# alibaba/open-simulator

Hardware: AMD Instinct MI355X
Metric: capacity-plan scenarios/sec (10k pods x ~1k nodes) (higher is better)
Workload: dtype u8 score table + u32 (gcd-normalised int64 quantities) + f64 (BalancedAllocation); 1 GPU; BASELINE config 3: 10000 pods x 488..1511 nodes, 1024 node counts x 4 pod orders = 4096 scenarios (4096 per GPU); scenarios_per_gpu=4096, pods=10000, node_pool=1512, kernel=score_table

## Files before the change

### open-simulator_amd/csrc/simon_hip.hip

```cpp
#include "../../include/simon_hip.h"
#include "simon_device.h"
#include "simon_wide.h"
#include "simon_table.h"
#include "simon_subset.h"
#include "simon_podsets.h"

#include <algorithm>
#include <cstdarg>
#include <cstdio>
#include <cstdlib>
#include <cstring>
#include <map>
#include <numeric>
#include <set>
#include <tuple>
#include <string>
#include <vector>

namespace simon {
struct PodRowF { double req_c, req_m, nz_c, nz_m; int32_t cls, preset, gate; uint32_t flags; };
struct FastScalars { int32_t mask_words, Cn, Cp, P, S; uint64_t g_cpu, g_mem; const uint32_t* pod_present; int32_t pp_words; };
struct FastLaunch {
    const uint32_t *a_cpu, *a_mem; const int32_t *a_pods, *ncls; const uint32_t *i_rq_cpu, *i_rq_mem, *i_nz_cpu, *i_nz_mem;
    const int32_t* i_npods; const PodRowF* pods; const int32_t* orders; const ScenarioDesc* scen; const int32_t* perm;
// ... 2624 lines not shown

static int run_table_batch(simon_ctx* c, const BatchRoute& r, bool want_placement, bool want_slices) {
    const int S = c->S, P = c->P;
    HIP_TRY(c, c->d_ws.ensure(c->ws_total));
    if (const char* fill = getenv("SIMON_WS_FILL"))
        HIP_TRY(c, hipMemsetAsync(c->d_ws.p, atoi(fill), c->ws_total, c->stream));
    if (want_placement) HIP_TRY(c, c->d_place_step.ensure((size_t)S * P));
    TableCold cold = table_cold(c, want_slices);
    TableLaunch f{};
    f.team = r.team; f.lds_ws = r.lds_ws; f.lds_x = r.lds_x;
    f.coarse = c->table_coarse; f.rest = c->rest; f.spread = c->spread; f.aff = c->rest && !c->aff_idx.empty(); f.nzeq = c->nzeq; f.has_pin = c->has_pin;
    f.sc = table_scalars(c, want_slices);
    const bool shared_pro = !c->no_shared_prologue && c->pro_nb > 0 && !c->has_ranks && !own_nodes(c) && table_shared_prologue(f);
    if (shared_pro) {
        HIP_TRY(c, c->d_pro_image.ensure(c->pro_bytes));
        cold.pro_image = c->d_pro_image.p; cold.pro_seg = c->d_pro_seg.p; cold.pro_nb = c->pro_nb; cold.pro_n = c->max_n;
    }
    if (c->table_prof) { HIP_TRY(c, c->d_table_prof.ensure((size_t)S * 24)); HIP_TRY(c, hipMemsetAsync(c->d_table_prof.p, 0, (size_t)S * 192, c->stream)); cold.prof = c->d_table_prof.p; }
    HIP_TRY(c, c->d_table_cold.ensure(sizeof cold));
    HIP_TRY(c, hipMemcpyAsync(c->d_table_cold.p, &cold, sizeof cold, hipMemcpyHostToDevice, c->stream));
    HIP_TRY(c, hipStreamSynchronize(c->stream));
    f.cold = reinterpret_cast<const TableCold*>(c->d_table_cold.p);
    f.cls_list = c->has_ranks ? c->d_rk_ids.p : c->d_cls_list.p; f.pods = c->d_podsC.p; f.orders = c->d_orders.p; f.perm = c->d_perm.p;
    f.place_step = want_placement ? c->d_place_step.p : nullptr;
    f.ws_off = c->d_ws_off.p; f.ws = c->d_ws.p;
    if (c->debug_route) {
        char own[64] = "none";
        if (const int lo = table_entries_own_size(f)) {
            int fits = 0;
            for (int s = 0; s < S; ++s) fits += c->scen_ni[s] <= 1024 * lo;
            if (c->no_size_dispatch) snprintf(own, sizeof own, "off");
            else snprintf(own, sizeof own, "%d of %d scenarios at %d", fits, S, lo);
        }
        fprintf(stderr, "[route] unit %s nzeq %d team %d prologue %s entries/lane %d (own size: %s)\n", table_unit_name(f), (int)f.nzeq, f.team,
                shared_pro ? "shared-image" : "per-scenario", table_entries_per_lane(f), own);
    }
    trace_segmented(c, "score-table kernel, ranked instantiation");
    if (int rc = timed_launch(c, [&] {
            if (shared_pro) HIP_TRY(c, launch_table_image(f, c->pro_nb, c->stream));
            HIP_TRY(c, launch_table(f, S, r.lds, c->stream));
            if (want_placement) HIP_TRY(c, launch_unpermute(c->d_place_step.p, c->d_inv_orders.p, c->d_scen.p, S, P, c->d_place.p, c->stream));
            return (int)SIMON_OK;
        })) return rc;
    return c->table_prof ? report_table_prof(c) : SIMON_OK;
}

static int run_fast_batch(simon_ctx* c, const BatchRoute& r, bool want_placement) {
    FastLaunch f{};
    fill_register_args(c, want_placement, f);
    f.pods = c->d_podsF.p;
    f.sc = FastScalars{(c->N + 63) / 64, c->Cn, c->Cp, c->P, c->S, c->g_cpu, c->g_mem, pod_rows(c), c->pod_W};
    return timed_launch(c, [&] { HIP_TRY(c, launch_fast(f, r.T, r.slots, c->has_mask, c->nzeq, r.lds, c->stream)); return (int)SIMON_OK; });
}

static int run_narrow_batch(simon_ctx* c, const BatchRoute& r, bool want_placement) {
    NarrowArgs a{};
    fill_register_args(c, want_placement, a);
    a.pods = c->d_podsN.p;
    a.mask_words = (c->N + 63) / 64; a.Cn = c->Cn; a.Cp = c->Cp; a.P = c->P; a.S = c->S;
    a.g_cpu = c->g_cpu; a.g_mem = c->g_mem;
    a.pod_present = pod_rows(c); a.pp_words = c->pod_W;
    return timed_launch(c, [&] { HIP_TRY(c, launch_narrow(a, r.T, r.slots, c->has_mask, c->rcp_div, r.lds, c->stream)); return (int)SIMON_OK; });
}

int simon_run_loaded(simon_ctx* c, int32_t want_placement) {
    if (!c) return SIMON_EINVAL;
    if (!c->staged || c->S <= 0) return fail(c, SIMON_ESTATE, "run_loaded: no scenarios loaded");
    if (c->evict_short >= 0 && !c->sub_on)
// ... 337 lines not shown
```

### open-simulator_amd/csrc/simon_table.h

```cpp
#pragma once

#include <hip/hip_runtime.h>
#include <stdint.h>

#include "simon_device.h"

namespace simon {

struct SigRow {
    double req_c, req_m;
    double nz_c, nz_m;
    int32_t cls;
    uint32_t flags;
    int32_t pad[2];
};
static_assert(sizeof(SigRow) == 48, "SigRow must be 48 bytes");

struct ShapeRow {
    double cap_c, cap_m;
    double rc_c, rc_m;
    double rc100_c, rc100_m;
};
static_assert(sizeof(ShapeRow) == 48, "ShapeRow must be 48 bytes");

// ... 92 lines not shown
constexpr int kTableMaxNodes = 4095;
constexpr int kTableMaxNodesCoarse = 8191;
constexpr int kTableMaxPadded = 4096;
constexpr int kTableMaxPaddedCoarse = 8192;
constexpr int kTableMaxSigs = 1023;
constexpr int kTableFastSigs = 384;
constexpr size_t kTableLdsPerCU = 160 * 1024;
constexpr int kTableMaxGpuSigs = 32;
constexpr int kTableMaxXres = 32;
constexpr int kTableMaxTerms = 120;
constexpr int kSpreadMaxZoneDom = 16;
constexpr int kSpreadMaxHostTerms = 4096, kSpreadMaxZoneTerms = 1024, kSpreadMaxZoneKeys = 3;
#ifndef SIMON_SPREAD_TAB_MAX
#define SIMON_SPREAD_TAB_MAX 512
#endif
constexpr int kSpreadTabMax = SIMON_SPREAD_TAB_MAX;
#ifndef SIMON_SPREAD_TAB_MAX2
#define SIMON_SPREAD_TAB_MAX2 2048
#endif
constexpr int kSpreadTabMax2 = SIMON_SPREAD_TAB_MAX2;
constexpr int kTeamWaves = 4;
constexpr int kTeamWavesMax = 16;
constexpr int kTableMaxClasses = 64;
constexpr int kTableMaxClassesSpread = 128;
constexpr int kTableMaxClassesPlain = 256;

constexpr int kLdsSecondTable = 0x100, kLdsTeam = 0x200, kLdsCn2 = 0x400;
size_t table_lds_bytes(int K, int ni_max, int Cn, bool coarse, bool rest, int nzk = -1);
size_t table_ws_bytes(int K, int ni, bool nzeq, bool coarse, int Cn, int M, int NZ, int TH = 0, int TZ = 0);
hipError_t launch_table(const TableLaunch& a, int n_blocks, size_t lds_bytes, hipStream_t st);
const char* table_unit_name(const TableLaunch& a);
int table_entries_per_lane(const TableLaunch& a);
int table_entries_own_size(const TableLaunch& a);
bool table_shared_prologue(const TableLaunch& a);
hipError_t launch_table_image(const TableLaunch& a, int nb, hipStream_t st);
inline size_t table_ldsx_bytes(int ni_max, int M) {
    return ((((size_t)(ni_max >> 4) * M * 2) + 127) & ~(size_t)127) + (((size_t)M * 4 + 127) & ~(size_t)127) + (((size_t)ni_max * 2 + 127) & ~(size_t)127);
}
hipError_t launch_unpermute(const int32_t* place_step, const int32_t* inv_orders, const ScenarioDesc* scen, int S, int P,
                            int32_t* placement, hipStream_t st);

}
```

### open-simulator_amd/csrc/simon_table.hip

```cpp
#ifndef SIMON_TABLE_BODY_PASS
#include "simon_table.h"

#include <algorithm>
#include <type_traits>

#ifdef SIMON_TABLE_PROFILE
#define TPROF_DECL unsigned long long tp_prev = __builtin_readcyclecounter(), tp_acc[24] = {0}; tp_acc[22] = tp_prev - tp_pro0; tp_acc[23] = tp_pro2;
#define TPROF_PROLOGUE_BEGIN const unsigned long long tp_pro0 = __builtin_readcyclecounter(); unsigned long long tp_pro2 = 0;
#define TPROF_TABLE_PASS_BEGIN tp_pro2 = __builtin_readcyclecounter()
#define TPROF_TABLE_PASS_END do { asm volatile("s_waitcnt vmcnt(0) lgkmcnt(0)" ::: "memory"); tp_pro2 = __builtin_readcyclecounter() - tp_pro2; } while (0)
#define TPROF(i) do { const unsigned long long t_ = __builtin_readcyclecounter(); tp_acc[i] += t_ - tp_prev; tp_prev = t_; } while (0)
#define TPROF_WAIT_LDS asm volatile("s_waitcnt lgkmcnt(0)" ::: "memory")
#define TPROF_WAIT_MEM asm volatile("s_waitcnt vmcnt(0)" ::: "memory")
#define TPROF_WAIT_STATE(n) asm volatile("s_waitcnt vmcnt(%0)" :: "n"(n) : "memory")
#else
#define TPROF_DECL
#define TPROF_PROLOGUE_BEGIN
#define TPROF_TABLE_PASS_BEGIN do { } while (0)
#define TPROF_TABLE_PASS_END do { } while (0)
#define TPROF(i) do { } while (0)
#define TPROF_WAIT_LDS do { } while (0)
#define TPROF_WAIT_MEM do { } while (0)
#define TPROF_WAIT_STATE(n) do { } while (0)
#endif
// ... 256 lines not shown
    int32_t* __restrict__ place_step, unsigned char* ws, const TableScalars sc) {
#endif
    GPtr<const TableCold> const cold = gp(cold_);
    GPtr<const int32_t> __restrict__ const ncls = gp(cold->ncls);
    GPtr<const int32_t> __restrict__ const cls_off = gp(cold->cls_off); GPtr<const int32_t> __restrict__ const clsprefix = gp(cold->clsprefix);
    GPtr<const int32_t> __restrict__ const a_pods = gp(cold->a_pods); GPtr<const uint32_t> __restrict__ const i_rq_cpu = gp(cold->i_rq_cpu);
    GPtr<const uint32_t> __restrict__ const i_rq_mem = gp(cold->i_rq_mem); GPtr<const uint32_t> __restrict__ const i_nz_cpu = gp(cold->i_nz_cpu);
    GPtr<const uint32_t> __restrict__ const i_nz_mem = gp(cold->i_nz_mem); GPtr<const int32_t> __restrict__ const i_npods = gp(cold->i_npods);
    const SigRow* __restrict__ const sigs = cold->sigs; const ShapeRow* __restrict__ const shapes = cold->shapes;
    const ScenarioDesc* __restrict__ const scen = cold->scen; GPtr<const uint64_t> __restrict__ const static_mask = gp(cold->static_mask);
    GPtr<const int32_t> __restrict__ const simon_raw = gp(cold->simon_raw);
    extern __shared__ __attribute__((aligned(16))) unsigned char smem[];
    const int Cn = sc.Cn, Cp = sc.Cp, P = sc.P, K = sc.K;
    constexpr int UB = COARSE ? 6 : 4;
    constexpr int UNIT = 1 << UB;
    constexpr unsigned UMASK = UNIT - 1;
    constexpr int KB = COARSE ? 13 : 12;
    constexpr unsigned PMASK = (1u << KB) - 1u;
    static_assert(!REST || COARSE, "the REST path is built on the two-level layout");
    constexpr bool kCls4 = CN2 && !REST && !SPREAD;
#ifdef SIMON_REST_CNT_HBM
    constexpr bool CNT_LDS = !COARSE;
#else
    constexpr bool CNT_LDS = (!COARSE || REST) && !kCls4;
#endif
#ifdef SIMON_TIE_SPECULATE
    constexpr bool TIE_FIRST = false;
#else
    constexpr bool TIE_FIRST = REST || MANY;
#endif
    constexpr bool kStraight = !REST && !SPREAD && !MANY;
    static_assert(!(kStraight && TIE_FIRST), "the straight-line cycle defines the winner's class and record index behind the assume's loads: nothing ahead of them may read dstar / res");
    static_assert(!kStraight || NW == 1, "team mode is SPREAD: a straight-line instantiation has no helper waves");
    constexpr bool kSharedPro = kSharedPrologueTU && !COARSE && !REST && !SPREAD && !MANY && !kCls4 && !RANKED && !LDSWS && NW == 1;
    static_assert(!MANY || (KQ == 2 && COARSE && !CN2 && !LDSX), "MANY = groups of 128 signatures on the two-level layout (since round 6 also under the REST select: its rows and counters are indexed by signature already)");
    constexpr int NG = MANY ? 2 : 0;
    static_assert(!SPREAD || COARSE, "SPREAD is built on the two-level layout");
    constexpr bool RS = REST && SPREAD;
    static_assert(!RS || (!LDSX && !CN2), "REST && SPREAD: <= 64 classes");
    static_assert(!(SPREAD && MANY) || NBQ == 2, "SPREAD with more than 128 signatures: the two-blocks-per-lane instantiations only");
    static_assert(NW == 1 || SPREAD, "team mode exists for the SPREAD instantiations");
    static_assert(!CN2 || (SPREAD && !MANY && !REST) || (REST && !LDSX && !SPREAD) || (!REST && !SPREAD && !COARSE && !MANY && !LDSWS), "CN2 = two node classes per lane in spread_select (<= 128 signatures) or in rest_select (rows in HBM); without rows and walks: 129 .. 256 classes on the one-level layout (simon_table_cls4.hip)");
    constexpr int TABMAX = CN2 ? kSpreadTabMax2 : kSpreadTabMax;
    const TCarve cv = tcarve(K, sc.ni_max, Cn, COARSE, REST, SPREAD ? (sc.NZK | ((sc.static_tables & kStSpreadAff) ? 0x100 : 0) | (NW > 1 ? 0x200 : 0) | (CN2 ? 0x400 : 0)) : -1, kCls4);
    const int TH = SPREAD ? sc.TH : 0, TZ = SPREAD ? sc.TZ : 0, NZK = SPREAD ? sc.NZK : 0;
    signed char* s_zdom = (signed char*)(smem + cv.zdom);
    unsigned short* s_stash = (unsigned short*)(smem + cv.stash);
    int* s_tabi = (int*)(smem + cv.tabi);
    int* s_tab = (int*)(smem + cv.tab);
    int* s_tot = NW > 1 ? (int*)(smem + cv.tab2) : s_tab;
    int* s_xch = (int*)(smem + cv.xch);
    const int M = REST ? sc.M : 0, G = REST ? sc.G : 0, X = REST ? sc.X : 0, NZ = REST ? sc.NZ : 0;
    const int nbp = cv.nbp;
    unsigned short* s_sn = (unsigned short*)(smem + cv.sn);
    int* s_cnt = (int*)(smem + cv.cnt);
    const ShapeRow* s_shape = (const ShapeRow*)(smem + cv.shape);
    auto shape_of = [&](int d) -> ShapeRow {
        if constexpr (kCls4) {
            const double* r = (const double*)(smem + cv.shape) + 4 * d;
            return ShapeRow{r[0], r[1], r[2], r[3], 100.0 * r[2], 100.0 * r[3]};
        } else return s_shape[d];
    };
    int* s_seg = (int*)(smem + cv.seg);
    int* s_tmp = (int*)(smem + cv.tmp);
    int2* s_ext = (int2*)(smem + cv.ext);

// ... 303 lines not shown
    if constexpr (SPREAD) {
        for (int i = tid; i < (NZK > 0 ? NZK : 1) * Cn; i += TT) s_zdom[i] = NZK > 0 ? gp(cold->cls_zdom)[i] : (signed char)0;
        for (size_t i = tid; i < ((size_t)TH * ni + 3) / 4; i += TT) ((unsigned*)g_hrow)[i] = 0u;
        for (int i = tid; i < TZ * 16; i += TT) g_zcnt[i] = 0u;
        for (int i = tid; i < TH; i += TT) g_hmax[i] = 0;
    }
    asm volatile("s_waitcnt vmcnt(0)" ::: "memory");
    if constexpr (NW > 1 || kCls4) __threadfence();
    __syncthreads();
    if constexpr (NW > 1) __threadfence();

    int kk[KQ];
    bool kvalid[KQ];
    double my_req_c[KQ], my_req_m[KQ], my_nz_c[KQ], my_nz_m[KQ];
    bool my_zero[KQ];
    int my_tc[KQ];
    unsigned my_add_c[KQ], my_add_m[KQ], my_addz_c[KQ], my_addz_m[KQ], koff[KQ];
    unsigned my_greq[KQ];
    int my_gnum[KQ];
    unsigned my_dirty = 0;
#pragma unroll
    for (int q = 0; q < KQ; ++q) {
        kvalid[q] = lane + 64 * q < K;
        kk[q] = kvalid[q] ? lane + 64 * q : 0;
        const SigRow r = sigs[kk[q]];
        my_req_c[q] = r.req_c; my_req_m[q] = r.req_m; my_nz_c[q] = r.nz_c; my_nz_m[q] = r.nz_m;
        my_zero[q] = r.flags & 1u;
        if constexpr (kCls4) my_tc[q] = r.cls;
        my_greq[q] = (unsigned)r.pad[0]; my_gnum[q] = kvalid[q] ? r.pad[1] : 0;
        my_add_c[q] = (unsigned)r.req_c; my_add_m[q] = (unsigned)r.req_m;
        my_addz_c[q] = (unsigned)r.nz_c; my_addz_m[q] = (unsigned)r.nz_m;
        koff[q] = (unsigned)kk[q] * KS;
    }
    for (int j = 0; j * 64 + lane < K; ++j) my_dirty |= 1u << j;
    int cb[NBQ], bcls[NBQ], binfo[NBQ];
#pragma unroll
    for (int q = 0; q < NBQ; ++q) {
        const int b = q * 64 + lane;
        cb[q] = (((int)(PMASK >> UB)) - b) << UB;
        bcls[q] = class_of_pos(b < nun ? b * UNIT : 0);
        binfo[q] = (cls_off[bcls[q]] - s_seg[bcls[q]] + 8192) | (bcls[q] << 16);
    }

    auto winner_info = [&](int bw) -> int {
        const int l = bw & 63, h = bw >> 6;
        int info = __builtin_amdgcn_readlane(binfo[0], l);
        if (NBQ > 1) { const int i1 = __builtin_amdgcn_readlane(binfo[NBQ > 1 ? 1 : 0], l); info = h == 1 ? i1 : info; }
        if (NBQ > 2) {
            const int i2 = __builtin_amdgcn_readlane(binfo[NBQ > 2 ? 2 : 0], l), i3 = __builtin_amdgcn_readlane(binfo[NBQ > 3 ? 3 : 0], l);
            info = h == 2 ? i2 : h == 3 ? i3 : info;
        }
        return info;
    };

    auto img_base = [&](GPtr<const TableCold> cc) -> size_t {
        return (size_t)__builtin_amdgcn_readfirstlane(gp(cc->img_slot)[s]) * (size_t)cc->img_stride;
    };
    auto class_term = [&](bool inb, int rawc, int c, int dd) -> int {
        const int lo = wave_min_i32(inb ? rawc : 0x7fffffff);
        const int hi = wave_max_i32(inb ? rawc : (int)0x80000000);
        const int range = hi >= lo ? hi - lo : 0;
        const double rr = range ? 1.0 / (double)range : 0.0;
        int term = (inb && range) ? 2 * (int)__builtin_fma((double)(rawc - lo) * 100.0, rr, 0.5 * rr) : 0;
        GPtr<const TableCold> cc = cold;
        asm volatile("" : "+s"(cc));
        if (sc.static_tables & kStNa) {
// ... 10 lines not shown
        }
        if (sc.static_tables & kStAdd) term += inb ? gp(cc->add_raw)[c * Cn + dd] : 0;
        if (sc.static_tables & kStImg) term += inb ? (int)gp(cc->img)[img_base(cc) + c * Cn + dd] : 0;
        return term;
    };
    auto class_term2 = [&](bool in0, bool in1, int raw0, int raw1, int c, int d0, int d1, int& t0, int& t1) {
        const int lo = min(wave_min_i32(in0 ? raw0 : 0x7fffffff), wave_min_i32(in1 ? raw1 : 0x7fffffff));
        const int hi = max(wave_max_i32(in0 ? raw0 : (int)0x80000000), wave_max_i32(in1 ? raw1 : (int)0x80000000));
        const int range = hi >= lo ? hi - lo : 0;
        const double rr = range ? 1.0 / (double)range : 0.0;
        t0 = (in0 && range) ? 2 * (int)__builtin_fma((double)(raw0 - lo) * 100.0, rr, 0.5 * rr) : 0;
        t1 = (in1 && range) ? 2 * (int)__builtin_fma((double)(raw1 - lo) * 100.0, rr, 0.5 * rr) : 0;
        GPtr<const TableCold> cc = cold;
        if (sc.static_tables & kStNa) {
            const int a0 = gp(cc->na_raw)[c * Cn + d0], a1 = gp(cc->na_raw)[c * Cn + d1];
            const int mx = max(wave_max_i32(in0 ? a0 : 0), wave_max_i32(in1 ? a1 : 0));
            const double r = mx ? 1.0 / (double)mx : 0.0;
            t0 += (in0 && mx) ? (int)__builtin_fma((double)a0 * 100.0, r, 0.5 * r) : 0;
            t1 += (in1 && mx) ? (int)__builtin_fma((double)a1 * 100.0, r, 0.5 * r) : 0;
        }
        if (sc.static_tables & kStTt) {
            const int a0 = gp(cc->tt_raw)[c * Cn + d0], a1 = gp(cc->tt_raw)[c * Cn + d1];
            const int mx = max(wave_max_i32(in0 ? a0 : 0), wave_max_i32(in1 ? a1 : 0));
            const double r = mx ? 1.0 / (double)mx : 0.0;
            t0 += in0 ? (mx ? 100 - (int)__builtin_fma((double)a0 * 100.0, r, 0.5 * r) : 100) : 0;
            t1 += in1 ? (mx ? 100 - (int)__builtin_fma((double)a1 * 100.0, r, 0.5 * r) : 100) : 0;
        }
        if (sc.static_tables & kStAdd) { t0 += in0 ? gp(cc->add_raw)[c * Cn + d0] : 0; t1 += in1 ? gp(cc->add_raw)[c * Cn + d1] : 0; }
        if (sc.static_tables & kStImg) {
            const size_t ib = img_base(cc);
            t0 += in0 ? (int)gp(cc->img)[ib + c * Cn + d0] : 0; t1 += in1 ? (int)gp(cc->img)[ib + c * Cn + d1] : 0;
        }
    };
    auto renormalise = [&](int k, int c) {
        if (kCls4 && Cn > 128) {
            int dq[4], cnq[4], rawq[4], tq[4];
            bool inq[4];
            int lo = 0x7fffffff, hi = (int)0x80000000;
#pragma unroll
            for (int g = 0; g < 4; ++g) {
                const bool v = g * 64 + lane < Cn;
                dq[g] = v ? g * 64 + lane : 0;
                cnq[g] = g_cnt[k * Cn + dq[g]];
                rawq[g] = simon_raw[c * Cn + dq[g]];
                inq[g] = v && cnq[g] > 0;
            }
#pragma unroll
            for (int g = 0; g < 4; ++g) { lo = min(lo, inq[g] ? rawq[g] : 0x7fffffff); hi = max(hi, inq[g] ? rawq[g] : (int)0x80000000); }
            lo = wave_min_i32(lo); hi = wave_max_i32(hi);
            if (lane == 0) s_ext[k] = make_int2(lo, hi);
            const int range = hi >= lo ? hi - lo : 0;
            const double rr = range ? 1.0 / (double)range : 0.0;
#pragma unroll
            for (int g = 0; g < 4; ++g) tq[g] = (inq[g] && range) ? 2 * (int)__builtin_fma((double)(rawq[g] - lo) * 100.0, rr, 0.5 * rr) : 0;
            GPtr<const TableCold> cc = cold;
            asm volatile("" : "+s"(cc));
            if (sc.static_tables & kStNa) {
                int a[4], mx = 0;
#pragma unroll
                for (int g = 0; g < 4; ++g) a[g] = gp(cc->na_raw)[c * Cn + dq[g]];
#pragma unroll
                for (int g = 0; g < 4; ++g) mx = max(mx, inq[g] ? a[g] : 0);
                mx = wave_max_i32(mx);
                const double r = mx ? 1.0 / (double)mx : 0.0;
#pragma unroll
                for (int g = 0; g < 4; ++g) tq[g] += (inq[g] && mx) ? (int)__builtin_fma((double)a[g] * 100.0, r, 0.5 * r) : 0;
// ... 64 lines not shown
        const int dd = lane < Cn ? lane : 0;
        const int cn = (lane < Cn) ? (!CNT_LDS ? g_cnt[k * Cn + dd] : s_cnt[k * Cn + dd]) : 0;
        const bool inb = cn > 0;
        const int rawc = simon_raw[c * Cn + dd];
        const int sn = class_term(inb, rawc, c, dd);
        if (lane < Cn) {
            s_tmp[dd] = sn - (int)s_sn[k * Cn + dd];
            s_sn[k * Cn + dd] = (unsigned short)sn;
        }
        }
        lead_sync();
        unsigned short* srow = s_sum + k * nbp;
#pragma unroll
        for (int q = 0; q < NBQ; ++q) {
            const int b = q * 64 + lane;
            if (b < nun) {
                const int delta = s_tmp[bcls[q]];
                const unsigned m = srow[b];
                if (m) srow[b] = (unsigned short)((int)m + delta * UNIT);
                if constexpr (COARSE) {
                    uint2* fp = (uint2*)(g_fine + ((size_t)b * K + k) * 4);
                    uint2 f = *fp;
                    auto shift2 = [&](unsigned w) -> unsigned {
                        const unsigned lo = w & 0xFFFFu, hi = w >> 16;
                        return ((lo ? (unsigned)((int)lo + delta * 16) : 0u) & 0xFFFFu) | ((hi ? (unsigned)((int)hi + delta * 16) : 0u) << 16);
                    };
                    f.x = shift2(f.x); f.y = shift2(f.y);
                    *fp = f;
                }
            }
        }
        lead_sync();
    };

    TPROF_DECL
    const uint2 my_gsig = REST ? ldg_u2(gp(cold->gsig) + (lane < G ? lane : 0)) : make_uint2(0, 0);
    unsigned my_xsig[5] = {0, 0, 0, 0, 0};
    if (REST && X > 0) {
        const int x = (lane >= 32 && lane - 32 < X) ? lane - 32 : 0;
        const uint4 q0 = ldg_u4(gp(cold->xsig) + (size_t)x * 8);
        my_xsig[0] = q0.x; my_xsig[1] = q0.y; my_xsig[2] = q0.z; my_xsig[3] = q0.w; my_xsig[4] = gp(cold->xsig)[(size_t)x * 8 + 4];
    }
    auto excluded = [&](int b, int nrows, int rowv, int gs, int xs, bool esc) -> unsigned {
        const unsigned short* xr = g_xm + b;
        unsigned bad = gs >= 0 ? (unsigned)xr[(size_t)gs * nblk] : 0u;
        if (xs >= 0) bad |= (unsigned)xr[(size_t)(G + xs) * nblk];
        for (int e = 0; e < nrows; ++e) {
            const unsigned ent = (unsigned)__builtin_amdgcn_readlane(rowv, e);
            const unsigned v = (unsigned)xr[(size_t)(ent & 0xFFFFu) * nblk];
            bad |= (AFF && (ent >> 31)) ? (esc ? 0u : (~v & 0xFFFFu)) : v;
        }
        return bad;
    };
    auto aff_escape = [&](int nrows, int rowv, unsigned rtv) -> bool {
        if (!AFF) return false;
        const bool inv = lane < nrows && ((unsigned)rowv >> 31);
        const bool self = __ballot(inv && (((unsigned)rowv >> 27) & 1u)) != 0ull;
        return self && __ballot(inv && rtv != 0u) == 0ull;
    };
    auto rest_select = [&](int k, int tc, int nrows, int rowv, int gs, int xs, bool esc, int& dstar, int& res) -> int {
        TPROF(11);
        const int dd = lane < Cn ? lane : 0;
        const int rawc = simon_raw[tc * Cn + dd];
        if (lane < Cn) s_tmp[lane] = 0;
        const bool v2 = CN2 && 64 + lane < Cn;
        const int dd2 = v2 ? 64 + lane : 0;
// ... 847 lines not shown
                res = -1;
                if (HAS_PIN && (segd ? __builtin_amdgcn_readfirstlane(gp(cc->rk_rank)[(size_t)s * (size_t)cc->N + pin]) < n : pin < n)) {
                    const int dp = __builtin_amdgcn_readfirstlane(gp(cc->ncls)[pin]);
                    const int rk = __builtin_amdgcn_readfirstlane(ranked ? gp(cc->rk_pos)[(size_t)s * (size_t)cc->N + pin] : gp(cc->rank)[pin]);
                    const int pp = __builtin_amdgcn_readfirstlane(s_seg[dp]) + rk;
                    const unsigned char byte = g_tile[tile_blk((unsigned)(pp >> 4)) + (unsigned)r_sig * KS + (unsigned)(pp & 15)];
                    bool clear = true;
                    if (REST && rw != 0) clear = !((__builtin_amdgcn_readfirstlane(excluded(pp >> 4, r_nrows, rowv, r_gs, r_xs, aff_escape(r_nrows, rowv, rtv))) >> (pp & 15)) & 1u);
                    if (byte != 0 && clear) { res = __builtin_amdgcn_readfirstlane(gp(cc->cls_off)[dp]) + rk; pstar = pp; dstar = dp; }
                }
            }
            if constexpr (kStraight) {
                if (pstar >= 0) assume(false, bound, pstar, dstar, res, 0u, m16q, e16q);
            }
        } else if (REST && __builtin_expect(rw != 0, 0) && !(RS && spread_pod)) {
            pstar = rest_select(r_sig, r_cls, r_nrows, rowv, r_gs, r_xs, aff_escape(r_nrows, rowv, rtv), dstar, res);
            TPROF(10);
            if (pstar < 0) res = -1;
        } else if (spread_pod) {
            const int k = r_sig;
            const unsigned dq = (unsigned)__builtin_amdgcn_readlane((int)my_dirty, k & 63);
            if ((dq >> (k >> 6)) & 1u) {
                renormalise(k, r_cls);
                if (lane == (k & 63)) my_dirty &= ~(1u << (k >> 6));
            }
            if constexpr (NW == 1) {
                if constexpr (RS) pstar = spread_select(k, r_cls, sp_soft, sp_match, sp_ipa, sp_hard, spv, spt, dstar, res, r_nrows, rowv, r_gs, r_xs, aff_escape(r_nrows, rowv, rtv));
                else pstar = spread_select(k, r_cls, sp_soft, sp_match, sp_ipa, sp_hard, spv, spt, dstar, res);
                TPROF(18);
                if (pstar < 0) res = -1;
            }
        } else {
            const int k = r_sig;
            const unsigned dq = (unsigned)__builtin_amdgcn_readlane((int)my_dirty, k & 63);
            if (__builtin_expect((dq >> (k >> 6)) & 1u, 0)) {
                renormalise(k, r_cls);
                if (lane == (k & 63)) my_dirty &= ~(1u << (k >> 6));
            }
            int ks = k;
            asm volatile("" : "+s"(ks));
            const unsigned short* srow = s_sum + ks * nbp;
            unsigned key = 0;
#pragma unroll
            for (int q = 0; q < NBQ; ++q) {
                const int b = q * 64 + lane;
                m16q[q] = srow[b < nun ? b : 0];
            }
#pragma unroll
            for (int q = 0; q < NBQ; ++q) {
                const unsigned m16 = m16q[q];
                if constexpr (kStraight) {
                    unsigned e;
                    asm("v_lshrrev_b32 %0, %2, %1" : "=v"(e) : "v"(m16), "n"(UB));
                    e16q[q] = e;
                    unsigned lo;
                    asm("v_and_or_b32 %0, %1, %2, %3" : "=v"(lo) : "v"(m16), "n"(UMASK), "v"(cb[q]));
                    key = max(key, (e << KB) | lo);
                } else {
                    key = max(key, (((m16 << (KB - UB)) & ~PMASK) | (unsigned)cb[q]) | (m16 & UMASK));
                }
            }
            TPROF_WAIT_LDS; TPROF(1);
            key = wave_max_u32(key);
            TPROF(2);
            if (__builtin_expect(key <= PMASK, 0)) {
                res = -1;
            } else {
                pstar = (int)(PMASK - (key & PMASK));
                top = key >> KB;
                scanned = true;
// ... 327 lines not shown
        else if constexpr (table_lo_entries(COARSE, RANKED, NBQ) != 0) return launch_kernel(table_kernel<true, Z, PIN, KQ, NBQ, COARSE, false, RANKED, false, MANY, false, 1, false, false, false, table_lo_entries(COARSE, RANKED, NBQ)>, a, n_blocks, 1, lds_bytes, st);
        else return launch_kernel(table_kernel<true, Z, PIN, KQ, NBQ, COARSE, false, RANKED, false, MANY, false>, a, n_blocks, 1, lds_bytes, st);
    }, a.nzeq, pin, table_kq(a), a.coarse, nbq, table_ranked(a), many);
}

enum class TableUnit { Team, Rs, Spread2, Spread, Lds, Rest2, RestLds, Rest, Cls4, Base };
static TableUnit table_route(const TableLaunch& a) {
    if (a.team > 1) return TableUnit::Team;
    if (a.spread && a.rest) return TableUnit::Rs;
    if (a.spread && a.sc.Cn > 64) return TableUnit::Spread2;
    if (a.spread) return TableUnit::Spread;
    if (a.lds_ws) return TableUnit::Lds;
    if (a.rest && a.sc.Cn > 64) return TableUnit::Rest2;
    if (a.rest && a.lds_x) return TableUnit::RestLds;
    if (a.rest) return TableUnit::Rest;
    if (!a.coarse && a.sc.Cn > 128) return TableUnit::Cls4;
    return TableUnit::Base;
}

static bool table_base_unit(const TableLaunch& a) { return table_route(a) == TableUnit::Base; }

const char* table_unit_name(const TableLaunch& a) {
    static const char* const names[] = {"simon_table_team4", "simon_table_rs", "simon_table_spread2", "simon_table_spread", "simon_table_lds",
                                        "simon_table_rest2", "simon_table_restlds", "simon_table_rest", "simon_table_cls4", "simon_table"};
    return names[(int)table_route(a)];
}

int table_entries_per_lane(const TableLaunch& a) {
    const TableUnit u = table_route(a);
    if (u == TableUnit::Cls4) return 4;
    if ((u == TableUnit::Team || u == TableUnit::Rs || u == TableUnit::Spread) && table_many(a)) return 2;
    return a.coarse ? table_nbq64(a).v : table_nbq16(a).v;
}
int table_entries_own_size(const TableLaunch& a) {
    return table_base_unit(a) ? table_lo_entries(a.coarse, table_ranked(a), table_entries_per_lane(a)) : 0;
}

hipError_t launch_table(const TableLaunch& a, int n_blocks, size_t lds_bytes, hipStream_t st) {
    switch (table_route(a)) {
        case TableUnit::Team: return a.team == kTeamWaves ? launch_table_team4(a, n_blocks, lds_bytes, st) : hipErrorInvalidValue;
        case TableUnit::Rs: return launch_table_rs(a, n_blocks, lds_bytes, st);
        case TableUnit::Spread2: return launch_table_spread2(a, n_blocks, lds_bytes, st);
        case TableUnit::Spread: return launch_table_spread(a, n_blocks, lds_bytes, st);
        case TableUnit::Lds: return launch_table_lds(a, n_blocks, lds_bytes, st);
        case TableUnit::Rest2: return launch_table_rest2(a, n_blocks, lds_bytes, st);
        case TableUnit::RestLds: return launch_table_rest_lds(a, n_blocks, lds_bytes, st);
        case TableUnit::Rest: return launch_table_rest(a, n_blocks, lds_bytes, st);
        case TableUnit::Cls4: return launch_table_cls4(a, n_blocks, lds_bytes, st);
        case TableUnit::Base: return launch_table_base(a, n_blocks, lds_bytes, st);
    }
    return hipErrorInvalidValue;
}
#endif

}
#endif
```

### open-simulator_amd/csrc/simon_table_assume.inc

```
            TPROF(3);
            auto tie_with_other_class = [&]() -> bool {
                bool other = false;
#pragma unroll
                for (int q = 0; q < NBQ; ++q) other |= ((kStraight ? e16q[q] : m16q[q] >> UB) == top) & (bcls[q] != dstar);
                return __ballot(other) != 0;
            };
            auto canonical_first = [&]() -> int {
#ifdef SIMON_TABLE_PROFILE
                tp_acc[7] += 1;
#endif
                unsigned key2 = 0;
                int canon[NBQ];
#pragma unroll
                for (int q = 0; q < NBQ; ++q) {
                    const int pq = (q * 64 + lane) * UNIT + (UNIT - 1) - (int)(m16q[q] & UMASK);
                    const bool tied = (m16q[q] >> UB) == top && q * 64 + lane < nun;
                    if constexpr (LDSX) canon[q] = tied ? (int)sx_canon[pq] : (int)PMASK;
                    else {
                    canon[q] = tied ? cls_list[rk_off + (unsigned)((binfo[q] & 0xFFFF) - 8192 + pq)] : (int)PMASK;
                    if (ranked && tied) canon[q] = gp(cold->rk_rank)[(size_t)s * (size_t)cold->N + canon[q]];
                    }
                }
#pragma unroll
                for (int q = 0; q < NBQ; ++q) {
// ... 144 lines not shown
            st.rq_m += add_m;
            st.freep -= 1u;
            double nzc = 0.0, nzm = 0.0;
            if (!NZEQ) {
                z.x += addz_c;
                z.y += addz_m;
                if (lane == 0) g_nz[pstar] = z;
                nzc = (double)z.x; nzm = (double)z.y;
            }
            if (lane == 0) *stp = st;
            const double rq_c = (double)st.rq_c, rq_m = (double)st.rq_m;
            TPROF(8);
            auto refresh_sig = [&](int k, bool valid, unsigned nb_raw,
                                   RowRef bytek, const uint4 Tk, const uint2 Fk, unsigned old, unsigned snk, int dirty_bit) {
                const unsigned nb = old ? nb_raw : 0u;
                if (valid && nb != old) {
                    byte_at(bytek, pos) = (unsigned char)nb;
                    const unsigned m = block_key16_patched<kStraight>(Tk, nb, pos, selA, selB, pos_c, c15);
                    const unsigned e16 = (m >> 4) ? m + (snk << 4) : 0u;
                    if constexpr (COARSE) {
                        const int j = blk & 3;
                        g_fine[((unsigned)(pstar >> 6) * (unsigned)K + (unsigned)k) * 4u + (unsigned)j] = (unsigned short)e16;
                        const unsigned keep = (j & 1) ? 0x0000FFFFu : 0xFFFF0000u, ins = e16 << ((j & 1) * 16);
                        const unsigned fx = (j & 2) ? Fk.x : ((Fk.x & keep) | ins);
                        const unsigned fy = (j & 2) ? ((Fk.y & keep) | ins) : Fk.y;
                        const unsigned cx = (((fx & 0xFFF0FFF0u) << 2) | (fx & 0x000F000Fu)) | 0x00200030u;
                        const unsigned cy = (((fy & 0xFFF0FFF0u) << 2) | (fy & 0x000F000Fu)) | 0x00000010u;
                        const unsigned mm = pkmax_t(cx, cy);
                        const unsigned c64 = max(mm & 0xFFFFu, mm >> 16);
                        s_sum[k * nbp + (pstar >> 6)] = (unsigned short)(c64 >= 64u ? c64 : 0u);
                    } else {
                        s_sum[k * nbp + blk] = (unsigned short)e16;
                    }
                    if (!nb) {
                        const int cidx = k * Cn + dstar;
                        int left;
                        if constexpr (!CNT_LDS) { left = g_cnt[cidx] - 1; g_cnt[cidx] = left; }
                        else { left = s_cnt[cidx] - 1; s_cnt[cidx] = left; }
                        bool rebase = left == 0;
                        if constexpr (kCls4) {
                            if (rebase && !(sc.static_tables & kStClassTerms)) {
                                const int raw = simon_raw[((KQ > 1 && dirty_bit == KQ - 1) ? my_tc[KQ - 1] : my_tc[0]) * Cn + dstar];
                                const int2 e = s_ext[k];
                                rebase = !(e.x < raw && raw < e.y);
                            }
                        }
                        if (rebase) my_dirty |= 1u << dirty_bit;
#ifdef SIMON_TABLE_DEBUG
                        printf("DBG s=%d step=%d CNT k=%d class=%d left=%d\n", s, i0 + il, k, dstar, left);
#endif
                    }
                }
            };
            unsigned nbq[KQ];
            nbq[0] = eval_node(my_req_c[0], my_req_m[0], my_nz_c[0], my_nz_m[0], my_zero[0], rq_c, rq_m, nzc, nzm, (int)st.freep, sh);
            if constexpr (KQ > 1) {
                if (sc.static_tables & kStTwins) nbq[KQ - 1] = nbq[0];
                else nbq[KQ - 1] = eval_node(my_req_c[KQ - 1], my_req_m[KQ - 1], my_nz_c[KQ - 1], my_nz_m[KQ - 1], my_zero[KQ - 1], rq_c, rq_m, nzc, nzm, (int)st.freep, sh);
            }
            if constexpr (kFoldable) {
                if (__builtin_expect(fold, 0)) {
#pragma unroll
                    for (int q = 0; q < KQ; ++q) nbq[q] = ((xfold[q] >> (kk[q] & 31)) & 1u) ? 0u : nbq[q];
                }
            }
            unsigned gu[8] = {0, 0, 0, 0, 0, 0, 0, 0};
            bool gbooked = false;
            if constexpr (kGpuFoldable) {
                if (__builtin_expect(gfold, 0)) {
                    unsigned greq = (unsigned)(hiq ? __builtin_amdgcn_readlane((int)my_greq[KQ - 1], sl) : __builtin_amdgcn_readlane((int)my_greq[0], sl));
                    int gnum = hiq ? __builtin_amdgcn_readlane(my_gnum[KQ - 1], sl) : __builtin_amdgcn_readlane(my_gnum[0], sl);
                    if (MANY && __builtin_expect(r_sig >= 64 * KQ, 0)) {
                        const SigRow rs = sigs[r_sig];
                        greq = (unsigned)rs.pad[0]; gnum = rs.pad[1];
                    }
                    if (gnum > 0 && !bound) {
                        unsigned (&u)[8] = gu;
                        u[0] = gfa.x; u[1] = gfa.y; u[2] = gfa.z; u[3] = gfa.w; u[4] = gfb.x; u[5] = gfb.y; u[6] = gfb.z; u[7] = gfb.w;
                        gbooked = true;
                        const unsigned long long booked = gpu_commit_t(u, gfc, gft, greq, gnum);
                        if (sc.static_tables & kStGpuSlices) {
                            const int pid = __builtin_amdgcn_readfirstlane(order[i0 + il]);
                            if (lane == 0) gp(cold->gpu_slices)[(size_t)s * (size_t)P + (size_t)pid] = booked;
                        }
                        if (lane == 0) {
                            *(uint4*)(g_fu + (size_t)pstar * 8) = make_uint4(u[0], u[1], u[2], u[3]);
                            *(uint4*)(g_fu + (size_t)pstar * 8 + 4) = make_uint4(u[4], u[5], u[6], u[7]);
                        }
#pragma unroll
                        for (int q = 0; q < KQ; ++q)
                            if (my_gnum[q] != 0 && !gpu_fits_t(u, gfc, gft, my_greq[q], my_gnum[q])) nbq[q] = 0u;
                    }
                }
            }
#pragma unroll
            for (int q = 0; q < KQ; ++q)
                refresh_sig(kk[q], kvalid[q], nbq[q], bytep[q], T[q], COARSE ? F[q] : make_uint2(0u, 0u),
                            oldq[q], snq[q], q);
            if constexpr (MANY) {
#pragma unroll
                for (int g = 0; g < NG; ++g) {
                    if (128 * (g + 1) < K) {
                        SigRow rg[KQ];
                        unsigned sng[KQ];
#pragma unroll
                        for (int q = 0; q < KQ; ++q) { rg[q] = sigs[kg[g][q]]; sng[q] = s_sn[kg[g][q] * Cn + dstar]; }
#pragma unroll
                        for (int q = 0; q < KQ; ++q)
                            refresh_sig(kg[g][q], 128 * (g + 1) + 64 * q + lane < K,
                                        ((fold && ((xfg[g][q] >> (kg[g][q] & 31)) & 1u)) ||
                                         (kGpuFoldable && gbooked && rg[q].pad[1] != 0 && !gpu_fits_t(gu, gfc, gft, (unsigned)rg[q].pad[0], rg[q].pad[1]))) ? 0u :
                                        eval_node(rg[q].req_c, rg[q].req_m, rg[q].nz_c, rg[q].nz_m, rg[q].flags & 1u, rq_c, rq_m, nzc, nzm, (int)st.freep, sh),
                                        rowg[g][q], Tg[g][q], Fg[g][q], oldg[g][q], sng[q], 2 * (g + 1) + q);
                    }
                }
                for (int g = NG; 128 * (g + 1) < K; ++g) {
#pragma unroll
                    for (int q = 0; q < KQ; ++q) {
                        const int kq = 128 * (g + 1) + 64 * q + lane;
                        const int kx = kq < K ? kq : 0;
                        const RowRef rowx = row_ref(tile_blk((unsigned)(pstar >> 4)) + (unsigned)kx * KS);
                        const uint4 Tx = row_vec(rowx);
                        const unsigned oldx = row_byte(rowx, pstar & 15);
                        const uint2 Fx = *(const uint2*)(g_fine + ((unsigned)(pstar >> 6) * (unsigned)K + (unsigned)kx) * 4u);
                        const unsigned xfx = fold ? gp(cold->foldx)[(unsigned)r_sig * KW + ((unsigned)kx >> 5)] : 0u;
                        const SigRow rx = sigs[kx];
                        const unsigned snx = s_sn[kx * Cn + dstar];
                        refresh_sig(kx, kq < K,
                                    ((fold && ((xfx >> (kx & 31)) & 1u)) ||
                                     (kGpuFoldable && gbooked && rx.pad[1] != 0 && !gpu_fits_t(gu, gfc, gft, (unsigned)rx.pad[0], rx.pad[1]))) ? 0u :
                                    eval_node(rx.req_c, rx.req_m, rx.nz_c, rx.nz_m, rx.flags & 1u, rq_c, rq_m, nzc, nzm, (int)st.freep, sh),
// ... 11 lines not shown
```

Before: 411,400 scenarios/s.

## Re-base score table eagerly at count-exhaustion events in straight-line kernel

For straight-line, non-coarse, non-class4 instantiations, signature renormalisation moves out of the per-pod dirty check. It now runs once up front for every signature, then again whenever a signature's count for a class drops to zero after a node's byte falls. This removes the per-step readlane and dirty-bit test on the hot selection path and the unconditional counter decrement. The cost is a ballot check every step plus renormalise calls at event time. A debug route line reporting the re-base mode and twins flag is also added.

```diff
diff --git a/open-simulator_amd/csrc/simon_hip.hip b/open-simulator_amd/csrc/simon_hip.hip
--- a/open-simulator_amd/csrc/simon_hip.hip
+++ b/open-simulator_amd/csrc/simon_hip.hip
@@ -2680,8 +2680,9 @@
             if (c->no_size_dispatch) snprintf(own, sizeof own, "off");
             else snprintf(own, sizeof own, "%d of %d scenarios at %d", fits, S, lo);
         }
-        fprintf(stderr, "[route] unit %s nzeq %d team %d prologue %s entries/lane %d (own size: %s)\n", table_unit_name(f), (int)f.nzeq, f.team,
-                shared_pro ? "shared-image" : "per-scenario", table_entries_per_lane(f), own);
+        fprintf(stderr, "[route] unit %s nzeq %d team %d prologue %s entries/lane %d (own size: %s) re-base %s twins %d\n", table_unit_name(f), (int)f.nzeq, f.team,
+                shared_pro ? "shared-image" : "per-scenario", table_entries_per_lane(f), own, table_rebase_at_event(f) ? "at-event" : "at-use",
+                (int)((f.sc.static_tables & kStTwins) != 0));
     }
     trace_segmented(c, "score-table kernel, ranked instantiation");
     if (int rc = timed_launch(c, [&] {
diff --git a/open-simulator_amd/csrc/simon_table.h b/open-simulator_amd/csrc/simon_table.h
--- a/open-simulator_amd/csrc/simon_table.h
+++ b/open-simulator_amd/csrc/simon_table.h
@@ -148,6 +148,7 @@
 const char* table_unit_name(const TableLaunch& a);
 int table_entries_per_lane(const TableLaunch& a);
 int table_entries_own_size(const TableLaunch& a);
+bool table_rebase_at_event(const TableLaunch& a);
 bool table_shared_prologue(const TableLaunch& a);
 hipError_t launch_table_image(const TableLaunch& a, int nb, hipStream_t st);
 inline size_t table_ldsx_bytes(int ni_max, int M) {
diff --git a/open-simulator_amd/csrc/simon_table.hip b/open-simulator_amd/csrc/simon_table.hip
--- a/open-simulator_amd/csrc/simon_table.hip
+++ b/open-simulator_amd/csrc/simon_table.hip
@@ -312,6 +312,7 @@
     constexpr bool kStraight = !REST && !SPREAD && !MANY;
     static_assert(!(kStraight && TIE_FIRST), "the straight-line cycle defines the winner's class and record index behind the assume's loads: nothing ahead of them may read dstar / res");
     static_assert(!kStraight || NW == 1, "team mode is SPREAD: a straight-line instantiation has no helper waves");
+    constexpr bool kEager = kStraight && !kCls4 && !COARSE;
     constexpr bool kSharedPro = kSharedPrologueTU && !COARSE && !REST && !SPREAD && !MANY && !kCls4 && !RANKED && !LDSWS && NW == 1;
     static_assert(!MANY || (KQ == 2 && COARSE && !CN2 && !LDSX), "MANY = groups of 128 signatures on the two-level layout (since round 6 also under the REST select: its rows and counters are indexed by signature already)");
     constexpr int NG = MANY ? 2 : 0;
@@ -681,6 +682,7 @@
         my_addz_c[q] = (unsigned)r.nz_c; my_addz_m[q] = (unsigned)r.nz_m;
         koff[q] = (unsigned)kk[q] * KS;
     }
+    if constexpr (!kEager)
     for (int j = 0; j * 64 + lane < K; ++j) my_dirty |= 1u << j;
     int cb[NBQ], bcls[NBQ], binfo[NBQ];
 #pragma unroll
@@ -757,6 +759,7 @@
             t0 += in0 ? (int)gp(cc->img)[ib + c * Cn + d0] : 0; t1 += in1 ? (int)gp(cc->img)[ib + c * Cn + d1] : 0;
         }
     };
+    auto sig_class = [&](int k) -> int { return __builtin_amdgcn_readfirstlane(gp(&sigs[k].cls)[0]); };
     auto renormalise = [&](int k, int c) {
         if (kCls4 && Cn > 128) {
             int dq[4], cnq[4], rawq[4], tq[4];
@@ -887,6 +890,9 @@
         }
         lead_sync();
     };
+    if constexpr (kEager) {
+        for (int k = 0; k < K; ++k) renormalise(k, sig_class(k));
+    }
 
     TPROF_DECL
     const uint2 my_gsig = REST ? ldg_u2(gp(cold->gsig) + (lane < G ? lane : 0)) : make_uint2(0, 0);
@@ -1800,10 +1806,12 @@
             }
         } else {
             const int k = r_sig;
-            const unsigned dq = (unsigned)__builtin_amdgcn_readlane((int)my_dirty, k & 63);
-            if (__builtin_expect((dq >> (k >> 6)) & 1u, 0)) {
-                renormalise(k, r_cls);
-                if (lane == (k & 63)) my_dirty &= ~(1u << (k >> 6));
+            if constexpr (!kEager) {
+                const unsigned dq = (unsigned)__builtin_amdgcn_readlane((int)my_dirty, k & 63);
+                if (__builtin_expect((dq >> (k >> 6)) & 1u, 0)) {
+                    renormalise(k, r_cls);
+                    if (lane == (k & 63)) my_dirty &= ~(1u << (k >> 6));
+                }
             }
             int ks = k;
             asm volatile("" : "+s"(ks));
@@ -2197,6 +2205,10 @@
     if ((u == TableUnit::Team || u == TableUnit::Rs || u == TableUnit::Spread) && table_many(a)) return 2;
     return a.coarse ? table_nbq64(a).v : table_nbq16(a).v;
 }
+bool table_rebase_at_event(const TableLaunch& a) {
+    const TableUnit u = table_route(a);
+    return u == TableUnit::Lds || (u == TableUnit::Base && !a.coarse);
+}
 int table_entries_own_size(const TableLaunch& a) {
     return table_base_unit(a) ? table_lo_entries(a.coarse, table_ranked(a), table_entries_per_lane(a)) : 0;
 }
diff --git a/open-simulator_amd/csrc/simon_table_assume.inc b/open-simulator_amd/csrc/simon_table_assume.inc
--- a/open-simulator_amd/csrc/simon_table_assume.inc
+++ b/open-simulator_amd/csrc/simon_table_assume.inc
@@ -200,6 +200,7 @@
                     } else {
                         s_sum[k * nbp + blk] = (unsigned short)e16;
                     }
+                    if constexpr (!kEager)
                     if (!nb) {
                         const int cidx = k * Cn + dstar;
                         int left;
@@ -265,6 +266,36 @@
             for (int q = 0; q < KQ; ++q)
                 refresh_sig(kk[q], kvalid[q], nbq[q], bytep[q], T[q], COARSE ? F[q] : make_uint2(0u, 0u),
                             oldq[q], snq[q], q);
+            if constexpr (kEager) {
+                bool gone = false;
+#pragma unroll
+                for (int q = 0; q < KQ; ++q) gone |= oldq[q] > (nbq[q] << 8);
+                if (__builtin_expect(__ballot(gone) != 0ull, 0)) {
+                    unsigned long long emptied[KQ];
+#pragma unroll
+                    for (int q = 0; q < KQ; ++q) {
+                        bool last = false;
+                        if (kvalid[q] && oldq[q] > (nbq[q] << 8)) {
+                            const int cidx = kk[q] * Cn + dstar;
+                            int left;
+                            if constexpr (!CNT_LDS) { left = g_cnt[cidx] - 1; g_cnt[cidx] = left; }
+                            else { left = s_cnt[cidx] - 1; s_cnt[cidx] = left; }
+                            last = left == 0;
+#ifdef SIMON_TABLE_DEBUG
+                            printf("DBG s=%d step=%d CNT k=%d class=%d left=%d\n", s, i0 + il, kk[q], dstar, left);
+#endif
+                        }
+                        emptied[q] = __ballot(last);
+                    }
+#pragma unroll
+                    for (int q = 0; q < KQ; ++q) {
+                        for (unsigned long long m = emptied[q]; m; m &= m - 1) {
+                            const int k = 64 * q + __builtin_ctzll(m);
+                            renormalise(k, sig_class(k));
+                        }
+                    }
+                }
+            }
             if constexpr (MANY) {
 #pragma unroll
                 for (int g = 0; g < NG; ++g) {
```

Result: faster. 420,100 scenarios/s (median of 6 runs) (+2.1%).
